# Caxson/mere-fusion

Hardware: AMD Instinct MI355X
Metric: lip-sync frames/sec @256x256 (higher is better)
Workload: dtype bf16x3+f16q; 1 GPU; MuseTalk step 256x256: pe(audio) + UNet(t=0) + VAE decode to uint8 frames, batch=8 latents + Whisper chunks per GPU, inputs resident in HBM (BASELINE.json configs[2]); assumed MuseTalk-v1 / sd-vae-ft-mse architecture, seeded random-init weights; batch_per_gpu=8, parallelism=1 independent replicas, sessions sharded by GPU, no collective

## Files before the change

include/merefusion.h:

```cpp
#ifndef MEREFUSION_H
#define MEREFUSION_H

#include <stddef.h>
#include <stdint.h>

#ifdef __cplusplus
extern "C" {
#endif

typedef enum mf_status {
    MF_OK = 0,
    MF_ERR_INVALID = -1,
    MF_ERR_HIP = -2,
    MF_ERR_NODEVICE = -3,
    MF_ERR_NOMEM = -4
} mf_status;

typedef enum mf_precision { MF_PREC_BF16 = 0, MF_PREC_BF16X3 = 1, MF_PREC_F16Q = 2 } mf_precision;

typedef struct mf_tensor {
    const char* name;
    const float* data;
    int ndim;
    int64_t shape[4];
// ... 35 lines not shown
    int transposed;
    int output_padding;
    int residual;
    int act;
    int in_h, in_w;
    int upsample;
    int pad_hi;
} mf_conv2d_desc;

int mf_conv2d_create(const mf_conv2d_desc* desc, const float* weight, const float* bias,
                     const float* bn_gamma, const float* bn_beta, const float* bn_mean,
                     const float* bn_var, int precision, mf_conv2d** out);
int mf_conv2d_forward(mf_conv2d* h, const float* x, float* y, int batch, void* stream);
int mf_conv2d_out_shape(const mf_conv2d* h, int* out_h, int* out_w);
int mf_conv2d_forward_stats(mf_conv2d* h, const float* x, float* y, int groups, double* stats, int batch, void* stream);
int mf_conv2d_time(mf_conv2d* h, int batch, int iters, float* ms, void* stream);
void mf_conv2d_destroy(mf_conv2d* h);
#define MF_CONV_FAMILY_IGEMM 0
#define MF_CONV_FAMILY_HALO 1
#define MF_CONV_FAMILY_HALO_W 2
#define MF_CONV_FAMILY_HALO_W_SPLIT 3
#define MF_CONV_FAMILY_TWIN 4
#define MF_CONV_FAMILY_THIN 5
#define MF_CONV_FAMILY_F16Q 6
#define MF_CONV_STATS_NONE 0
#define MF_CONV_STATS_EPILOGUE 1
#define MF_CONV_STATS_COMBINE 2
#define MF_CONV_STATS_PASS 3
int mf_conv2d_launch_config(const mf_conv2d* h, int batch, int stats_groups, int* info, int n);
int mf_conv2d_pin_config(mf_conv2d* h, int batch, int bm, int bn, int wgm, int wgn, int nsplit, int ld);
// ... 251 lines not shown
```

mere-fusion_amd/_lib.py:

```python
import ctypes as C
import os

HERE = os.path.dirname(os.path.abspath(__file__))
LIB_PATH = os.path.join(HERE, "libmerefusion_hip.so")

MF_PREC_BF16 = 0
MF_PREC_BF16X3 = 1
MF_PREC_F16Q = 2
PRECISIONS = {"bf16": MF_PREC_BF16, "bf16x3": MF_PREC_BF16X3, "f16q": MF_PREC_F16Q}


class MfTensor(C.Structure):
    _fields_ = [("name", C.c_char_p), ("data", C.c_void_p), ("ndim", C.c_int), ("shape", C.c_int64 * 4)]


class MfConv2dDesc(C.Structure):
    _fields_ = [(n, C.c_int) for n in (
        "cin", "cout", "kh", "kw", "stride_h", "stride_w", "pad_h", "pad_w", "transposed",
        "output_padding", "residual", "act", "in_h", "in_w", "upsample", "pad_hi")]


class MfUnetConfig(C.Structure):
    _fields_ = [("in_channels", C.c_int), ("out_channels", C.c_int), ("n_blocks", C.c_int),
                ("block_out_channels", C.c_int * 4), ("layers_per_block", C.c_int), ("cross_attention_dim", C.c_int),
# ... 51 lines not shown
    "mf_abi_version": (C.c_int, []),
    "mf_wav2lip_create": (C.c_int, [C.POINTER(MfTensor), C.c_int, C.c_int, C.POINTER(C.c_void_p)]),
    "mf_wav2lip_forward": (C.c_int, [C.c_void_p, C.c_void_p, C.c_void_p, C.c_void_p, C.c_int, C.c_void_p]),
    "mf_wav2lip_forward_u8": (C.c_int, [C.c_void_p, C.c_void_p, C.c_void_p, C.c_void_p, C.c_int, C.c_void_p]),
    "mf_wav2lip_read_tap": (C.c_int, [C.c_void_p, C.c_char_p, C.c_void_p, C.c_int, C.c_void_p]),
    "mf_wav2lip_num_launches": (C.c_int, [C.c_void_p, C.c_int]),
    "mf_wav2lip_launch_info": (C.c_int, [C.c_void_p, C.c_int, C.c_int, C.c_char_p, C.c_int, C.c_char_p, C.c_int,
                                        C.POINTER(C.c_double)]),
    "mf_wav2lip_profile": (C.c_int, [C.c_void_p, C.c_void_p, C.c_void_p, C.c_void_p, C.c_int, C.c_int,
                                     C.POINTER(C.c_float), C.c_void_p]),
    "mf_wav2lip_tune": (C.c_int, [C.c_void_p, C.c_int, C.c_void_p]),
    "mf_wav2lip_destroy": (None, [C.c_void_p]),
    "mf_conv2d_create": (C.c_int, [C.POINTER(MfConv2dDesc)] + [C.c_void_p] * 6 + [C.c_int, C.POINTER(C.c_void_p)]),
    "mf_conv2d_forward": (C.c_int, [C.c_void_p, C.c_void_p, C.c_void_p, C.c_int, C.c_void_p]),
    "mf_conv2d_forward_stats": (C.c_int, [C.c_void_p, C.c_void_p, C.c_void_p, C.c_int, C.c_void_p, C.c_int, C.c_void_p]),
    "mf_conv2d_out_shape": (C.c_int, [C.c_void_p, C.POINTER(C.c_int), C.POINTER(C.c_int)]),
    "mf_conv2d_time": (C.c_int, [C.c_void_p, C.c_int, C.c_int, C.POINTER(C.c_float), C.c_void_p]),
    "mf_conv2d_destroy": (None, [C.c_void_p]),
    "mf_conv2d_launch_config": (C.c_int, [C.c_void_p, C.c_int, C.c_int, C.POINTER(C.c_int), C.c_int]),
    "mf_conv2d_pin_config": (C.c_int, [C.c_void_p] + [C.c_int] * 7),
    "mf_whisper_create": (C.c_int, [C.POINTER(MfTensor), C.c_int, C.c_int, C.c_int, C.POINTER(C.c_void_p)]),
    "mf_whisper_dims": (C.c_int, [C.c_void_p, C.POINTER(C.c_int), C.POINTER(C.c_int), C.POINTER(C.c_int)]),
    "mf_whisper_log_mel": (C.c_int, [C.c_void_p, C.c_void_p, C.c_int, C.c_void_p, C.c_void_p]),
    "mf_whisper_encode_audio": (C.c_int, [C.c_void_p, C.c_void_p, C.c_int, C.c_void_p, C.c_void_p]),
    "mf_whisper_set_batch": (C.c_int, [C.c_void_p, C.c_int]),
    "mf_whisper_encode_windows": (C.c_int, [C.c_void_p, C.c_void_p, C.c_int, C.c_int, C.c_int, C.c_void_p, C.c_void_p]),
    "mf_whisper_destroy": (None, [C.c_void_p]),
    "mf_wav2vec2_create": (C.c_int, [C.POINTER(MfWav2Vec2Config), C.POINTER(MfTensor), C.c_int, C.c_int, C.c_int, C.c_int, C.POINTER(C.c_void_p)]),
    "mf_wav2vec2_frames": (C.c_int, [C.c_void_p, C.POINTER(C.c_int), C.POINTER(C.c_int)]),
    "mf_wav2vec2_forward": (C.c_int, [C.c_void_p, C.c_void_p, C.c_int, C.c_int, C.c_void_p, C.c_void_p]),
# ... 137 lines not shown
```

mere-fusion_amd/csrc/mf_conv.h:

```cpp
#pragma once
#include "mf_common.h"
#include <map>
#include <vector>
#include <utility>

struct ActBuf {
    int C = 0, H = 0, W = 0, halo = 0;
    bf16_t* hi = nullptr;
    bf16_t* lo = nullptr;
    int Hp() const { return H + 2 * halo; }
    int Wp() const { return W + 2 * halo; }
    int64_t per_batch() const { return (int64_t)Hp() * Wp() * C; }
};

struct ActView {
    const ActBuf* buf = nullptr;
    int coff = 0;
    int C = 0;
};

#define MF_MAX_PHASE 9

struct ConvPhase {
    int goff_begin;
// ... 13 lines not shown
    const int* goff;
    int M, N, Npad;
    int HqWq, Wq;
    uint32_t dv_hw_mul, dv_hw_shr, dv_w_mul, dv_w_shr;
    uint32_t dv_t_mul, dv_t_shr, dv_s_mul, dv_s_shr;
    int64_t xb; int xi, xj;
    int64_t yb; int yi, yj;
    int64_t rb; int ri, rj;
    int act;
    int res_after_act;
    int tiles_m, tiles_n;
    unsigned long long* dbg;
    int m_fastest;
    int ld;
    int wide_store;
    int goff_total;
    int zgroups, zheads;
    int64_t zx_b, zx_h, zw, zy_b, zy_h;
    float* ws;
    int64_t ws_split, wsb; int wsi, wsj;
    double* gn_out; int gn_out_cpg, gn_out_groups;
    double* ln_out; const double* ln_in; const float* ln_cs; float ln_inv_c, ln_eps;
    ConvPhase ph[MF_MAX_PHASE];
};

struct HaloArgs {
    const bf16_t* x_hi; const bf16_t* x_lo;
    const bf16_t* w_hi; const bf16_t* w_lo;
    const float* bias;
    const bf16_t* r_hi; const bf16_t* r_lo;
// ... 23 lines not shown
    int pad, in_halo, in_hp, in_wp, x_ld;
    int64_t xb, yb; int yi, yj;
    int act;
};
bool mf_thin_supported(int k, int stride, int cin, int cout);
int mf_thin_nks(int k, int cin);
void mf_thin_pack(const float* w, const float* scale, int cout, int cin, int k, bool x3, std::vector<bf16_t>& dst);
int mf_thin_launch(const ThinArgs& a, int k, int stride, int cin, int cout, bool x3, hipStream_t s);
HaloTile mf_halo_pick_tile(int H, int W, int N, int batch, int cin = 0);
int mf_halo_launch(const HaloArgs& a, const HaloTile& t, bool x3, hipStream_t s);
HaloTile mf_halo_w_pick_tile(int H, int W, int N, int batch, int cin = 0);
int mf_halo_w_launch(const HaloArgs& a, const HaloTile& t, bool x3, hipStream_t s, int phase = -1);
struct ConvTile { int bm, bn, wgm, wgn, nsplit; };
struct ConvTuned { ConvTile tile; int ld; };

struct ConvPlan {
    mf_conv2d_desc d{};
    int precision = 0;
    int cin_pad = 0;
    int out_h = 0, out_w = 0;
    int Hq = 0, Wq = 0;
    int nphase = 1;
    int Npad = 0;
    int BK = 64;
    bf16_t* w_hi = nullptr;
    bf16_t* w_lo = nullptr;
    float* bias = nullptr;
    int* goff = nullptr;
    double* out_stats = nullptr; int out_stats_groups = 0;
    const float* ln_gamma = nullptr; const float* ln_beta = nullptr;
    float* ln_cs = nullptr; const double* ln_in = nullptr; float ln_eps = 1e-5f;
    double* ln_out = nullptr;
// ... 22 lines not shown
    ConvPhase ph[MF_MAX_PHASE]{};
    int goff_total = 0;
    int bound_in_ld = -1, bound_in_wp = -1;
    std::map<int, ConvTuned> tuned;
};

int mf_conv_plan_create(ConvPlan* p, const mf_conv2d_desc& d, const float* weight, const float* bias,
                        const float* bn_gamma, const float* bn_beta, const float* bn_mean,
                        const float* bn_var, int precision);
void mf_conv_plan_destroy(ConvPlan* p);

int mf_conv_bind(ConvPlan* p, const ActBuf& in);

struct ConvLaunchCfg { int family; ConvTile tile; int ld, bk, nphase, stats; bool pinned; };
int mf_conv_resolve(const ConvPlan* p, int batch, int tokens, int stats_groups, ConvLaunchCfg* c);
bool mf_conv_tuned_valid(const ConvTuned& c, int precision, int act);
int mf_conv_pin(ConvPlan* p, int batch, const ConvTuned& c);
void mf_conv_kernel_name(const ConvPlan* p, int batch, char* buf, int cap);
ConvTile mf_conv_pick_tile(const ConvPlan* p, int batch);
int mf_conv_tune(ConvPlan* p, const ActView& in, const ActView& out, const ActView& res, int batch, hipStream_t stream);
int mf_conv_tune_lookup(ConvPlan* p, const ActView& in, int batch);
bool mf_autotune_enabled();
double mf_conv_flops(const ConvPlan* p, int batch);

struct GroupedGemm {
    const bf16_t* x_hi; const bf16_t* x_lo; int64_t zx_b, zx_h; int x_row;
    bf16_t* y_hi; bf16_t* y_lo; int64_t zy_b, zy_h; int y_row;
    int M, groups, heads;
};
int mf_gemm_grouped_launch(ConvPlan* p, const GroupedGemm& g, hipStream_t stream);
// ... 8 lines not shown
```

mere-fusion_amd/csrc/mf_conv.hip:

```cpp
#include "mf_conv.h"
#include <dlfcn.h>
#include <cmath>
#include <cstdlib>
#include <cstring>
#include <algorithm>
#include <map>
#include <set>
#include <string>
#include <type_traits>

typedef __attribute__((ext_vector_type(8))) __bf16 bf16x8;
typedef __attribute__((ext_vector_type(4))) float f32x4;
typedef __attribute__((ext_vector_type(4))) unsigned int u32x4;
typedef __attribute__((ext_vector_type(8))) _Float16 f16x8;
typedef __attribute__((ext_vector_type(8))) int i32x8;
typedef __attribute__((ext_vector_type(4))) int i32x4;

template <int BK>
__device__ __forceinline__ int swz(int row) {
    return BK == 32 ? (((row >> 2) & 1) << 1) : (((row >> 1) & 3) << 1);
}
template <int BK>
__device__ __forceinline__ int tile_off(int row, int kg) {
    return row * (BK * 2) + ((kg ^ swz<BK>(row)) << 4);
// ... 86 lines not shown
template <int BM, int BN, int BK, bool X3>
constexpr int igemm_ring() {
    constexpr int stage = (BM + BN) * BK * 2 * (X3 ? 2 : 1);
    constexpr int by_lds = (144 * 1024) / stage;
    return by_lds < 8 ? by_lds : 8;
}

#ifndef MF_PW_NPW
#define MF_PW_NPW 4
#endif
template <int BM, int BN, int BK>
constexpr int igemm_producers() {
    constexpr int rpc = 1024 / (BK * 2), pch = (BM + rpc - 1) / rpc, wch = (BN + rpc - 1) / rpc;
    return (pch % MF_PW_NPW == 0 && wch % MF_PW_NPW == 0) ? MF_PW_NPW : 4;
}
template <int BM, int BN, int WGM, int WGN, bool X3, int BK, int NST, int LD = 0, bool Q = false>
__global__ __launch_bounds__((WGM * WGN + (LD == 3 ? igemm_producers<BM, BN, BK>() : 0)) * 64) void k_conv_igemm(const ConvArgs a) {
    static_assert(!Q || X3, "the f16 + FP6 format has two planes");
    constexpr int NW = WGM * WGN;
    constexpr int NS = LD == 3 ? igemm_producers<BM, BN, BK>() : NW;
    constexpr int NT = (NW + (LD == 3 ? NS : 0)) * 64;
    static_assert(NW == 4 || NW == 8, "4 or 8 waves per workgroup");
    static_assert(BK == 32 || BK == 64, "LDS tile depth");
    static_assert(NST == 2, "two LDS stages (deeper rings halved the workgroups per CU and measured slower)");
    constexpr int KG = BK / 8;
    constexpr int ROWB = BK * 2;
    constexpr int RPC = 1024 / ROWB;
    constexpr int NP = X3 ? 2 : 1;
    constexpr int WTM = BM / WGM, WTN = BN / WGN;
    constexpr int FM = WTM / 16, FN = WTN / 16;
    static_assert(FM >= 1 && FN >= 1, "wave tile must hold a 16x16 fragment");
    constexpr int P_BYTES = BM * ROWB, W_BYTES = BN * ROWB;
    constexpr int PLANE = P_BYTES + W_BYTES;
// ... 150 lines not shown
#pragma unroll
                for (int j = 0; j < FM; ++j) {
                    if (X3) {
                        acc[i][j] = __builtin_amdgcn_mfma_f32_16x16x32_bf16(wf[NP - 1][i], pf[0][j], acc[i][j], 0, 0, 0);
                        acc[i][j] = __builtin_amdgcn_mfma_f32_16x16x32_bf16(wf[0][i], pf[NP - 1][j], acc[i][j], 0, 0, 0);
                    }
                    acc[i][j] = __builtin_amdgcn_mfma_f32_16x16x32_bf16(wf[0][i], pf[0][j], acc[i][j], 0, 0, 0);
                }
        }
    };
    auto compute = [&](int s) __attribute__((always_inline)) {
        const char* base = smem + s * STAGE;
        compute_at(base, PLANE, base + P_BYTES, PLANE);
    };

    __syncthreads();
    if (dbg && threadIdx.x == 0) dbg[1] = __builtin_amdgcn_s_memtime();
    const int nk = kt_end - kt_begin;
    if constexpr (LD == 3) {
        constexpr int NPI = (NPC + NWC) * NP;
        static_assert(PCH % NS == 0 && WCH >= NS, "producer-wave path: every producer issues the same number of pieces per stage (weight pieces: duplicates fill up)");
#ifndef MF_PW_LEAD
        constexpr int LEAD = DR >= 5 ? 2 : 1;
#else
        constexpr int LEAD = MF_PW_LEAD;
#endif
        static_assert((DR - 1 - LEAD) * NPI <= 63 && DR - 1 - LEAD >= 0, "vmcnt immediate");
        if (wave >= NW) {
            if (nk > 0) {
                const int pre = nk < DR - 1 ? nk : DR - 1;
                for (int d = 0; d < pre; ++d) stage(kt_begin + d, d);
                if (pre == DR - 1) wait_vm<(DR - 1 - LEAD) * NPI>(); else wait_vm<0>();
                __builtin_amdgcn_s_barrier();
// ... 27 lines not shown
        auto mma = [&](auto bufc) __attribute__((always_inline)) {
            constexpr int b = decltype(bufc)::value;
#pragma unroll
            for (int i = 0; i < FN; ++i)
#pragma unroll
                for (int j = 0; j < FM; ++j) {
                    if (X3) {
                        acc[i][j] = __builtin_amdgcn_mfma_f32_16x16x32_bf16(wfr[b][NP - 1][i], pfr[b][0][j], acc[i][j], 0, 0, 0);
                        acc[i][j] = __builtin_amdgcn_mfma_f32_16x16x32_bf16(wfr[b][0][i], pfr[b][NP - 1][j], acc[i][j], 0, 0, 0);
                    }
                    acc[i][j] = __builtin_amdgcn_mfma_f32_16x16x32_bf16(wfr[b][0][i], pfr[b][0][j], acc[i][j], 0, 0, 0);
                }
        };
        using B0 = std::integral_constant<int, 0>;
        using B1 = std::integral_constant<int, 1>;
        if (nk > 0 && LEAD == 1) {
            __syncthreads();
            int slot = 0;
            for (int i = 0; i < nk; ++i) {
                ldf(B0{}, slot, 0);
                if constexpr (KK == 2) ldf(B1{}, slot, 1);
                mma(B0{});
                if constexpr (KK == 2) mma(B1{});
                slot = slot + 1 == DR ? 0 : slot + 1;
                __syncthreads();
            }
        } else if (nk > 0) {
            __syncthreads();
            ldf(B0{}, 0, 0);
            int slot = 0;
// ... 14 lines not shown
                    mma(B0{});
                    slot = nslot;
                    __syncthreads();
                    if (i + 1 < nk) {
                        nslot = slot + 1 == DR ? 0 : slot + 1;
                        if (i + 2 < nk) ldf(B0{}, nslot, 0);
                        mma(B1{});
                        slot = nslot;
                        __syncthreads();
                    }
                }
            }
        }
    } else if constexpr (LD != 0) {
        static_assert(LD == 2, "register-staged tiles: one LDS stage");
        u32x4 rp[NP][NPC], rw[NP][NWC];
        auto gload = [&](int kt) __attribute__((always_inline)) {
#pragma unroll
            for (int i = 0; i < NPC; ++i) {
                const int c = wave + NW * i;
                if (PCH % NW == 0 || c < PCH) {
                    const bf16_t* src = xp[i] + s_goff[kt * KG + p_kg[i]];
                    rp[0][i] = *reinterpret_cast<const u32x4*>(src);
                    if (X3) rp[NP - 1][i] = *reinterpret_cast<const u32x4*>(src + x_delta);
                }
            }
#pragma unroll
            for (int i = 0; i < NWC; ++i) {
                const int c = wave + NW * i;
                if (WCH % NW == 0 || c < WCH) {
                    const bf16_t* src = BK == 64 ? wp[i] + kt * w_kstep : wp[i] + (kt >> 1) * w_kstep + (kt & 1) * 32;
                    rw[0][i] = *reinterpret_cast<const u32x4*>(src);
                    if (X3) rw[NP - 1][i] = *reinterpret_cast<const u32x4*>(src + w_delta);
                }
            }
        };
        auto lstore = [&](int s) __attribute__((always_inline)) {
            char* base = smem + s * STAGE + lane * 16;
#pragma unroll
            for (int i = 0; i < NPC; ++i) {
                const int c = wave + NW * i;
                if (PCH % NW == 0 || c < PCH) {
                    *reinterpret_cast<u32x4*>(base + c * 1024) = rp[0][i];
                    if (X3) *reinterpret_cast<u32x4*>(base + PLANE + c * 1024) = rp[NP - 1][i];
                }
            }
#pragma unroll
            for (int i = 0; i < NWC; ++i) {
                const int c = wave + NW * i;
                if (WCH % NW == 0 || c < WCH) {
                    *reinterpret_cast<u32x4*>(base + P_BYTES + c * 1024) = rw[0][i];
                    if (X3) *reinterpret_cast<u32x4*>(base + PLANE + P_BYTES + c * 1024) = rw[NP - 1][i];
                }
            }
        };
        {
            if (nk > 0) gload(kt_begin);
            for (int kt = kt_begin; kt < kt_end; ++kt) {
                if (kt > kt_begin) __syncthreads();
                lstore(0);
                if (kt + 1 < kt_end) gload(kt + 1);
                __syncthreads();
                compute(0);
            }
        }
    } else {
        if (nk > 0) {
            stage(kt_begin, 0);
            __syncthreads();
            for (int kt = kt_begin; kt < kt_end; ++kt) {
                const int s = (kt - kt_begin) & 1;
                if (kt + 1 < kt_end) stage(kt + 1, s ^ 1);
                compute(s);
                __syncthreads();
            }
        }
    }

    if (dbg && threadIdx.x == 0) dbg[2] = __builtin_amdgcn_s_memtime();
    if (a.ws) {
#pragma unroll
        for (int j = 0; j < FM; ++j) {
            const int m = m0 + pm0 + j * 16 + fr;
// ... 1 lines not shown
            const int b = mf_fdiv(m, a.dv_hw_mul, a.dv_hw_shr);
            const int rem = m - b * a.HqWq;
            const int qi = mf_fdiv(rem, a.dv_w_mul, a.dv_w_shr), qj = rem - qi * a.Wq;
            float* wo = a.ws + (int64_t)blockIdx.y * a.ws_split + (int64_t)b * a.wsb + (int64_t)qi * a.wsi +
                        (int64_t)qj * a.wsj + ph.ws_off;
#pragma unroll
            for (int i = 0; i < FN; ++i) {
                const int c = n0 + cn0 + i * 16 + fk * 4;
                if (c >= a.N) continue;
                *reinterpret_cast<float4*>(wo + c) = make_float4(acc[i][j][0], acc[i][j][1], acc[i][j][2], acc[i][j][3]);
            }
        }
        if (dbg && threadIdx.x == 0) dbg[3] = __builtin_amdgcn_s_memtime();
        return;
    }
    float4 bq[FN];
#pragma unroll
    for (int i = 0; i < FN; ++i) {
        int c = n0 + cn0 + i * 16 + fk * 4;
        c = c < a.Npad - 3 ? c : a.Npad - 4;
        bq[i] = *reinterpret_cast<const float4*>(a.bias + c);
    }
    const int ACT = a.act;
    if (a.ln_in) {
#pragma unroll
        for (int j = 0; j < FM; ++j) {
            const int m = m0 + pm0 + j * 16 + fr;
            const bool row_ok = m < a.M;
            const int mc = row_ok ? m : a.M - 1;
            const int b = mf_fdiv(mc, a.dv_hw_mul, a.dv_hw_shr);
            const int rem = mc - b * a.HqWq;
            const int qi = mf_fdiv(rem, a.dv_w_mul, a.dv_w_shr), qj = rem - qi * a.Wq;
            const int64_t yo = zy + (int64_t)b * a.yb + (int64_t)qi * a.yi + (int64_t)qj * a.yj + ph.y_off;
            const double2 sq = *reinterpret_cast<const double2*>(a.ln_in + 2 * (int64_t)mc);
            const double mean = sq.x * (double)a.ln_inv_c, var = sq.y * (double)a.ln_inv_c - mean * mean;
            const float mu = (float)mean, rs = (float)(1.0 / sqrt((var > 0.0 ? var : 0.0) + (double)a.ln_eps));
            auto quad = [&](int i, float (&v)[4]) __attribute__((always_inline)) {
                int c = n0 + cn0 + i * 16 + fk * 4;
                c = c < a.Npad - 3 ? c : a.Npad - 4;
                const float4 cs = *reinterpret_cast<const float4*>(a.ln_cs + c);
                float t0 = acc[i][j][0] - mu * cs.x, t1 = acc[i][j][1] - mu * cs.y, t2 = acc[i][j][2] - mu * cs.z, t3 = acc[i][j][3] - mu * cs.w;
                asm volatile("" : "+v"(t0), "+v"(t1), "+v"(t2), "+v"(t3));
                v[0] = rs * t0 + bq[i].x; v[1] = rs * t1 + bq[i].y; v[2] = rs * t2 + bq[i].z; v[3] = rs * t3 + bq[i].w;
                asm volatile("" : "+v"(v[0]), "+v"(v[1]), "+v"(v[2]), "+v"(v[3]));
            };
            auto pack = [&](const float (&v)[4], uint2& hi2, uint2& lo2) __attribute__((always_inline)) {
                uint32_t h[4];
#pragma unroll
                for (int e = 0; e < 4; ++e) h[e] = f2bf(v[e]);
                hi2 = make_uint2(h[0] | (h[1] << 16), h[2] | (h[3] << 16));
                if (X3) {
                    uint32_t l[4];
#pragma unroll
                    for (int e = 0; e < 4; ++e) l[e] = f2bf(v[e] - bf2f(h[e]));
                    lo2 = make_uint2(l[0] | (l[1] << 16), l[2] | (l[3] << 16));
// ... 101 lines not shown
        }
    } else {
        constexpr int RB = (FM * FN >= 32) ? 16 : 32;
        constexpr int JG = (FM * FN * NP <= RB) ? FM : (RB / (FN * NP) >= 1 ? RB / (FN * NP) : 1);
        const bool has_res = a.r_hi != nullptr;
        const bool after = a.res_after_act;
        constexpr bool ST = NW == 4 && FM * FN < 16;
        float gs[ST ? FN : 1][4], gq[ST ? FN : 1][4];
#pragma unroll
        for (int i = 0; i < (ST ? FN : 1); ++i)
#pragma unroll
            for (int e = 0; e < 4; ++e) { gs[i][e] = 0.f; gq[i][e] = 0.f; }
#pragma unroll
        for (int j0 = 0; j0 < FM; j0 += JG) {
            uint2 rh[JG][FN], rl[JG][FN];
            if (has_res) {
#pragma unroll
                for (int jj = 0; jj < JG; ++jj) {
                    if (j0 + jj >= FM) break;
                    int m = m0 + pm0 + (j0 + jj) * 16 + fr;
                    m = m < a.M ? m : a.M - 1;
                    const int b = mf_fdiv(m, a.dv_hw_mul, a.dv_hw_shr);
                    const int rem = m - b * a.HqWq;
                    const int qi = mf_fdiv(rem, a.dv_w_mul, a.dv_w_shr), qj = rem - qi * a.Wq;
                    const int64_t ro = (int64_t)b * a.rb + (int64_t)qi * a.ri + (int64_t)qj * a.rj;
#pragma unroll
                    for (int i = 0; i < FN; ++i) {
                        int c = n0 + cn0 + i * 16 + fk * 4;
                        c = c < a.N ? c : 0;
                        rh[jj][i] = *reinterpret_cast<const uint2*>(a.r_hi + ro + c);
                        if (X3) rl[jj][i] = *reinterpret_cast<const uint2*>(a.r_lo + ro + c);
// ... 330 lines not shown

static EpiDiv epi_div(const ConvArgs& e, int Ho, int Wo) {
    EpiDiv d{};
    const int nq = ((e.act == 5 ? e.N >> 1 : e.N) >> 2);
    const int nq_all = e.N >> 2, cols = nq_all < 256 ? nq_all : 256;
    mf_fastdiv((uint32_t)nq, &d.nq_mul, &d.nq_shr);
    mf_fastdiv((uint32_t)Wo, &d.w_mul, &d.w_shr);
    mf_fastdiv((uint32_t)Ho, &d.h_mul, &d.h_shr);
    mf_fastdiv((uint32_t)(e.gn_out_cpg > 0 ? e.gn_out_cpg : 1), &d.g_mul, &d.g_shr);
    mf_fastdiv((uint32_t)(cols > 0 ? cols : 1), &d.c_mul, &d.c_shr);
    return d;
}

namespace {

template <int BM, int BN, int WGM, int WGN, bool X3, int BK, int NST, int LD = 0, bool Q = false>
int launch_cfg_n(const ConvArgs& a, int nphase, int nsplit, int goff_max, hipStream_t s) {
    static bool attr_done = false;
    auto kern = k_conv_igemm<BM, BN, WGM, WGN, X3, BK, NST, LD, Q>;
    if (!attr_done) {
        MF_HIP(hipFuncSetAttribute(reinterpret_cast<const void*>(kern),
                                   hipFuncAttributeMaxDynamicSharedMemorySize, 160 * 1024));
        attr_done = true;
    }
    size_t lds = (size_t)(LD == 2 ? 1 : NST) * (BM + BN) * BK * 2 * (X3 ? 2 : 1) + (size_t)goff_max * 4;
    if constexpr (LD == 3) {
        lds = (size_t)igemm_ring<BM, BN, BK, X3>() * (BM + BN) * BK * 2 * (X3 ? 2 : 1) + (size_t)goff_max * 4;
        if (lds > 160 * 1024) { mf_set_error("conv: producer-wave tile %dx%d needs %zu bytes of LDS", BM, BN, lds); return MF_ERR_INVALID; }
    }
    dim3 grid(a.tiles_m * a.tiles_n, nsplit, a.zgroups ? a.zgroups : nphase);
    ConvArgs b = a;
    mf_fastdiv((uint32_t)(a.m_fastest ? a.tiles_m : a.tiles_n), &b.dv_t_mul, &b.dv_t_shr);
    mf_fastdiv((uint32_t)nsplit, &b.dv_s_mul, &b.dv_s_shr);
    hipLaunchKernelGGL(kern, grid, dim3((WGM * WGN + (LD == 3 ? igemm_producers<BM, BN, BK>() : 0)) * 64), lds, s, b);
// ... 890 lines not shown
    {
        const int n_out = p->d.act == 5 ? p->d.cout / 2 : p->d.cout;
        a.wide_store = out.coff % 8 == 0 && ob.C % 8 == 0 && n_out % 8 == 0 && p->d.cout % 16 == 0;
    }
    a.goff_total = p->goff_total;
    int goff_max = 0;
    for (int ph = 0; ph < p->nphase; ++ph) {
        a.ph[ph] = p->ph[ph];
        a.ph[ph].y_off = ((int64_t)p->phase_oy[ph] * ob.Wp() + p->phase_ox[ph]) * ob.C;
        a.ph[ph].ws_off = ((int64_t)p->phase_oy[ph] * p->out_w + p->phase_ox[ph]) * a.N;
        goff_max = std::max(goff_max, p->ph[ph].ngroups);
    }

    const ConvTile tc = cfg.tile;
    a.ld = cfg.ld;
    a.tiles_m = cdiv(a.M, tc.bm); a.tiles_n = cdiv(a.N, tc.bn);
    {
        const int64_t w_elems = (int64_t)a.Npad * p->ph[0].KT * 64 * p->nphase;
        const int64_t x_elems = (int64_t)batch * ib.H * ib.W * in.C;
        a.m_fastest = w_elems > x_elems;
        static const bool dbg_times = mf_debug_has("times");
        if (dbg_times) {
            static unsigned long long* dbg_buf = nullptr;
            if (!dbg_buf) MF_HIP(hipMalloc(&dbg_buf, (size_t)4 * 65536 * sizeof(unsigned long long)));
            a.dbg = (int64_t)a.tiles_m * a.tiles_n * tc.nsplit * p->nphase <= 65536 ? dbg_buf : nullptr;
        }
    }
    if (tc.nsplit > 1) {
        const int64_t per_split = (int64_t)batch * p->out_h * out_w_eff * a.N;
        const int64_t need = per_split * tc.nsplit;
// ... 50 lines not shown
    }
    if (tc.nsplit > 1 && p->prof_mid) MF_HIP(hipEventRecord(p->prof_mid, stream));
    if (tc.nsplit > 1) {
        ConvArgs e = a;
        e.yi = ob.Wp() * ob.C; e.yj = ob.C;
        const int64_t total = (int64_t)batch * p->out_h * out_w_eff * ((a.act == 5 ? a.N / 2 : a.N) / 4);
        MF_REQUIRE(total < 0x7fffffffll, "conv: split-K combine over %lld channel quads (32-bit thread index)", (long long)total);
        if (tokens == 0 && launch_combine_stats(p, e, tc.nsplit, p->out_h, out_w_eff, batch, stream)) *stats_done = true;
        else hipLaunchKernelGGL(k_splitk_epilogue, dim3((unsigned)((total + 255) / 256)), dim3(256), 0, stream, e,
                                tc.nsplit, p->out_h, out_w_eff, (int)total, epi_div(e, p->out_h, out_w_eff));
        MF_HIP(hipGetLastError());
    }
    return MF_OK;
}

int mf_gemm_grouped_launch(ConvPlan* p, const GroupedGemm& g, hipStream_t stream) {
    MF_REQUIRE(!p->halo && p->nphase == 1 && p->bound_in_ld > 0, "grouped gemm: plan must be a bound mf_gemm_plan_create shell");
    const bool x3 = p->precision == MF_PREC_BF16X3;
    ConvArgs a{};
    a.x_hi = g.x_hi; a.x_lo = x3 ? g.x_lo : nullptr;
    a.w_hi = p->w_hi; a.w_lo = p->w_lo; a.bias = p->bias; a.goff = p->goff;
    a.M = g.M; a.N = p->d.cout; a.Npad = p->Npad;
    a.HqWq = g.M; a.Wq = g.M;
    mf_fastdiv((uint32_t)a.HqWq, &a.dv_hw_mul, &a.dv_hw_shr); mf_fastdiv((uint32_t)a.Wq, &a.dv_w_mul, &a.dv_w_shr);
    a.xb = 0; a.xi = 0; a.xj = g.x_row;
    a.y_hi = g.y_hi; a.y_lo = x3 ? g.y_lo : nullptr;
    a.yb = 0; a.yi = 0; a.yj = g.y_row;
    a.act = 0;
    a.ld = -1;
    a.goff_total = p->goff_total;
    a.ph[0] = p->ph[0];
    a.zgroups = g.groups; a.zheads = g.heads;
    a.zx_b = g.zx_b; a.zx_h = g.zx_h; a.zy_b = g.zy_b; a.zy_h = g.zy_h;
    a.zw = (int64_t)p->ph[0].KT * p->Npad * 64;
    const int M = g.M, N = a.N;
    int rc = MF_ERR_INVALID;
#define MF_GCASE(BM, BN, WGM, WGN)                                                         \
    { a.tiles_m = cdiv(M, BM); a.tiles_n = cdiv(N, BN);                                    \
      rc = launch_prec<BM, BN, WGM, WGN>(a, 1, 1, p->ph[0].ngroups, x3, false, stream); }
    if (N <= 16) MF_GCASE(128, 16, 4, 1)
    else if (N <= 32) MF_GCASE(128, 32, 4, 1)
    else if (M <= 16) MF_GCASE(16, 64, 1, 4)
    else if (cdiv(M, 128) * cdiv(N, 128) * g.groups >= 512 && N % 128 == 0) MF_GCASE(128, 128, 2, 2)
    else if (cdiv(M, 128) * cdiv(N, 64) * g.groups >= 512) MF_GCASE(128, 64, 2, 2)
// ... 302 lines not shown
```

mere-fusion_amd/csrc/mf_conv_api.hip:

```cpp
#include "mf_conv.h"
#include "mf_aux.h"
#include <memory>
#include <algorithm>

static int out_channels(const mf_conv2d_desc& d) { return d.act == 5 ? d.cout / 2 : d.cout; }

struct mf_conv2d {
    ConvPlan plan;
    ActBuf in, out;
    int cap = 0;
    ~mf_conv2d() {
        mf_conv_plan_destroy(&plan);
        for (ActBuf* b : {&in, &out}) {
            if (b->hi) (void)hipFree(b->hi);
            if (b->lo) (void)hipFree(b->lo);
        }
    }
};

extern "C" int mf_conv2d_create(const mf_conv2d_desc* desc, const float* weight, const float* bias,
                                const float* bn_gamma, const float* bn_beta, const float* bn_mean,
                                const float* bn_var, int precision, mf_conv2d** out) {
    MF_REQUIRE(desc && weight && out, "conv2d_create: null argument");
    MF_REQUIRE((bn_gamma != nullptr) == (bn_beta != nullptr) && (bn_gamma != nullptr) == (bn_mean != nullptr) &&
// ... 42 lines not shown
    ActView res = h->plan.d.residual ? ActView{&h->in, 0, h->plan.d.cout} : ActView{};
    if ((rc = mf_conv_launch(&h->plan, in, out, res, batch, s))) return rc;
    return mf_act_to_nchw(out, y, batch, s);
}

extern "C" int mf_conv2d_forward_stats(mf_conv2d* h, const float* x, float* y, int groups, double* stats, int batch, void* stream) {
    MF_REQUIRE(h && stats && groups > 0 && groups <= 64 && h->plan.d.act != 5 && h->plan.d.cout % groups == 0 && h->plan.d.cout % 8 == 0,
               "conv2d_forward_stats: needs cout %% groups == 0, cout %% 8 == 0, groups <= 64, no GEGLU");
    MF_HIP(hipMemsetAsync(stats, 0, (size_t)batch * groups * 2 * sizeof(double), (hipStream_t)stream));
    h->plan.out_stats = stats; h->plan.out_stats_groups = groups;
    const int rc = mf_conv2d_forward(h, x, y, batch, stream);
    h->plan.out_stats = nullptr; h->plan.out_stats_groups = 0;
    return rc;
}

extern "C" int mf_conv2d_time(mf_conv2d* h, int batch, int iters, float* ms, void* stream) {
    MF_REQUIRE(h && ms, "conv2d_time: null argument");
    MF_REQUIRE(batch > 0 && batch <= h->cap && iters > 0, "conv2d_time: run mf_conv2d_forward at this batch first");
    hipStream_t s = (hipStream_t)stream;
    ActView in{&h->in, 0, h->in.C}, out{&h->out, 0, out_channels(h->plan.d)};
    ActView res = h->plan.d.residual ? ActView{&h->in, 0, h->plan.d.cout} : ActView{};
    hipEvent_t e0, e1;
    MF_HIP(hipEventCreate(&e0)); MF_HIP(hipEventCreate(&e1));
    MF_HIP(hipEventRecord(e0, s));
    for (int i = 0; i < iters; ++i) {
        int rc = mf_conv_launch(&h->plan, in, out, res, batch, s);
        if (rc) return rc;
    }
    MF_HIP(hipEventRecord(e1, s));
    MF_HIP(hipEventSynchronize(e1));
// ... 6 lines not shown

extern "C" int mf_conv2d_out_shape(const mf_conv2d* h, int* out_h, int* out_w) {
    MF_REQUIRE(h && out_h && out_w, "conv2d_out_shape: null argument");
    *out_h = h->plan.out_h; *out_w = h->plan.out_w;
    return MF_OK;
}

extern "C" void mf_conv2d_destroy(mf_conv2d* h) { delete h; }

extern "C" int mf_conv2d_launch_config(const mf_conv2d* h, int batch, int stats_groups, int* info, int n) {
    MF_REQUIRE(h && info && n >= 11 && batch > 0 && stats_groups >= 0, "conv2d_launch_config: needs a handle, batch > 0, stats_groups >= 0 and room for 11 ints");
    ConvLaunchCfg c;
    if (const int rc = mf_conv_resolve(&h->plan, batch, 0, stats_groups, &c)) return rc;
    const int v[11] = {c.family, c.tile.bm, c.tile.bn, c.tile.wgm, c.tile.wgn, c.tile.nsplit, c.ld, c.bk, c.nphase, c.stats, c.pinned ? 1 : 0};
    std::copy(v, v + 11, info);
    return MF_OK;
}

extern "C" int mf_conv2d_pin_config(mf_conv2d* h, int batch, int bm, int bn, int wgm, int wgn, int nsplit, int ld) {
    MF_REQUIRE(h && batch > 0, "conv2d_pin_config: null handle or batch <= 0");
    return mf_conv_pin(&h->plan, batch, ConvTuned{ConvTile{bm, bn, wgm, wgn, nsplit}, ld});
}
```

Baseline: 452.4 frames/s.

## Prefetch epilogue operands during the igemm mainloop and split register-staged loads

Adds an EPF variant of the implicit-GEMM conv kernel that loads bias, layernorm statistics and residual tiles into registers during the last mainloop stage, so the epilogue no longer waits on those global loads. For register-staged (LD==2) forms it also issues the first weight load before the initial barrier and splits activation and weight loads. The variant is enabled by default through an env switch and is limited to 4-wave forms with small fragment counts. It raises register pressure, which may cut occupancy. New LN-conv API entry points are added for testing.

```diff
diff --git a/include/merefusion.h b/include/merefusion.h
--- a/include/merefusion.h
+++ b/include/merefusion.h
@@ -73,6 +73,9 @@
 int mf_conv2d_forward(mf_conv2d* h, const float* x, float* y, int batch, void* stream);
 int mf_conv2d_out_shape(const mf_conv2d* h, int* out_h, int* out_w);
 int mf_conv2d_forward_stats(mf_conv2d* h, const float* x, float* y, int groups, double* stats, int batch, void* stream);
+int mf_conv2d_create_ln(const mf_conv2d_desc* desc, const float* weight, const float* bias, const float* ln_gamma, const float* ln_beta, float eps,
+                        int precision, mf_conv2d** out);
+int mf_conv2d_forward_ln(mf_conv2d* h, const float* x, const double* stats, float* y, int batch, void* stream);
 int mf_conv2d_time(mf_conv2d* h, int batch, int iters, float* ms, void* stream);
 void mf_conv2d_destroy(mf_conv2d* h);
 #define MF_CONV_FAMILY_IGEMM 0
diff --git a/mere-fusion_amd/_lib.py b/mere-fusion_amd/_lib.py
--- a/mere-fusion_amd/_lib.py
+++ b/mere-fusion_amd/_lib.py
@@ -89,6 +89,8 @@
     "mf_conv2d_create": (C.c_int, [C.POINTER(MfConv2dDesc)] + [C.c_void_p] * 6 + [C.c_int, C.POINTER(C.c_void_p)]),
     "mf_conv2d_forward": (C.c_int, [C.c_void_p, C.c_void_p, C.c_void_p, C.c_int, C.c_void_p]),
     "mf_conv2d_forward_stats": (C.c_int, [C.c_void_p, C.c_void_p, C.c_void_p, C.c_int, C.c_void_p, C.c_int, C.c_void_p]),
+    "mf_conv2d_create_ln": (C.c_int, [C.POINTER(MfConv2dDesc)] + [C.c_void_p] * 4 + [C.c_float, C.c_int, C.POINTER(C.c_void_p)]),
+    "mf_conv2d_forward_ln": (C.c_int, [C.c_void_p, C.c_void_p, C.c_void_p, C.c_void_p, C.c_int, C.c_void_p]),
     "mf_conv2d_out_shape": (C.c_int, [C.c_void_p, C.POINTER(C.c_int), C.POINTER(C.c_int)]),
     "mf_conv2d_time": (C.c_int, [C.c_void_p, C.c_int, C.c_int, C.POINTER(C.c_float), C.c_void_p]),
     "mf_conv2d_destroy": (None, [C.c_void_p]),
diff --git a/mere-fusion_amd/csrc/mf_conv.h b/mere-fusion_amd/csrc/mf_conv.h
--- a/mere-fusion_amd/csrc/mf_conv.h
+++ b/mere-fusion_amd/csrc/mf_conv.h
@@ -1,5 +1,6 @@
 #pragma once
 #include "mf_common.h"
+#include <cstdlib>
 #include <map>
 #include <vector>
 #include <utility>
@@ -51,6 +52,7 @@
     int m_fastest;
     int ld;
     int wide_store;
+    int epi_pf;
     int goff_total;
     int zgroups, zheads;
     int64_t zx_b, zx_h, zw, zy_b, zy_h;
@@ -104,8 +106,11 @@
 struct ConvTile { int bm, bn, wgm, wgn, nsplit; };
 struct ConvTuned { ConvTile tile; int ld; };
 
+inline bool mf_epi_prefetch_env() { const char* e = getenv("MF_EPI_PREFETCH"); return !(e && *e && atoi(e) == 0); }
+
 struct ConvPlan {
     mf_conv2d_desc d{};
+    bool epi_prefetch = mf_epi_prefetch_env();
     int precision = 0;
     int cin_pad = 0;
     int out_h = 0, out_w = 0;
@@ -158,6 +163,7 @@
 
 struct ConvLaunchCfg { int family; ConvTile tile; int ld, bk, nphase, stats; bool pinned; };
 int mf_conv_resolve(const ConvPlan* p, int batch, int tokens, int stats_groups, ConvLaunchCfg* c);
+bool mf_conv_epf_runs(const ConvPlan* p, const ConvLaunchCfg& c);
 bool mf_conv_tuned_valid(const ConvTuned& c, int precision, int act);
 int mf_conv_pin(ConvPlan* p, int batch, const ConvTuned& c);
 void mf_conv_kernel_name(const ConvPlan* p, int batch, char* buf, int cap);
diff --git a/mere-fusion_amd/csrc/mf_conv.hip b/mere-fusion_amd/csrc/mf_conv.hip
--- a/mere-fusion_amd/csrc/mf_conv.hip
+++ b/mere-fusion_amd/csrc/mf_conv.hip
@@ -124,9 +124,16 @@
     constexpr int rpc = 1024 / (BK * 2), pch = (BM + rpc - 1) / rpc, wch = (BN + rpc - 1) / rpc;
     return (pch % MF_PW_NPW == 0 && wch % MF_PW_NPW == 0) ? MF_PW_NPW : 4;
 }
-template <int BM, int BN, int WGM, int WGN, bool X3, int BK, int NST, int LD = 0, bool Q = false>
+constexpr bool igemm_epf_form(int bm, int bn, int wgm, int wgn, bool x3, int bk, int ld, bool q) {
+    return wgm * wgn == 4 && !q && (bm / wgm / 16) * (bn / wgn / 16) <= 8 && !(ld == 2 && !x3 && bm == 128 && bn == 64) && !(ld != 3 && x3 && bk == 32);
+}
+template <int BM, int BN, int WGM, int WGN, bool X3, int BK, int LD, bool Q>
+constexpr bool igemm_epf() { return igemm_epf_form(BM, BN, WGM, WGN, X3, BK, LD, Q); }
+
+template <int BM, int BN, int WGM, int WGN, bool X3, int BK, int NST, int LD = 0, bool Q = false, bool EPF = false>
 __global__ __launch_bounds__((WGM * WGN + (LD == 3 ? igemm_producers<BM, BN, BK>() : 0)) * 64) void k_conv_igemm(const ConvArgs a) {
     static_assert(!Q || X3, "the f16 + FP6 format has two planes");
+    static_assert(!EPF || igemm_epf<BM, BN, WGM, WGN, X3, BK, LD, Q>(), "epilogue operand prefetch: forms that keep their workgroups per CU only");
     constexpr int NW = WGM * WGN;
     constexpr int NS = LD == 3 ? igemm_producers<BM, BN, BK>() : NW;
     constexpr int NT = (NW + (LD == 3 ? NS : 0)) * 64;
@@ -307,9 +314,83 @@
         compute_at(base, PLANE, base + P_BYTES, PLANE);
     };
 
+    float4 bq[FN];
+    constexpr int PF_LN = 4 * FM + 4 * FN, PF_RES = 2 * FM * FN * NP;
+    uint32_t pf[EPF ? (PF_LN > PF_RES ? PF_LN : PF_RES) : 1];
+    static_assert(!EPF || FM * FN * NP <= 16, "the prefetched residual is one row group of the general epilogue");
+    auto epi_prefetch = [&]() __attribute__((always_inline)) {
+        if constexpr (EPF) {
+            if (a.ws) return;
+#pragma unroll
+            for (int i = 0; i < FN; ++i) {
+                int c = n0 + cn0 + i * 16 + fk * 4;
+                c = c < a.Npad - 3 ? c : a.Npad - 4;
+                bq[i] = *reinterpret_cast<const float4*>(a.bias + c);
+                if (a.ln_in) {
+                    const uint4 cs = *reinterpret_cast<const uint4*>(a.ln_cs + c);
+                    pf[4 * FM + 4 * i] = cs.x; pf[4 * FM + 4 * i + 1] = cs.y; pf[4 * FM + 4 * i + 2] = cs.z; pf[4 * FM + 4 * i + 3] = cs.w;
+                }
+            }
+            if (a.ln_in) {
+#pragma unroll
+                for (int j = 0; j < FM; ++j) {
+                    const int m = m0 + pm0 + j * 16 + fr;
+                    const int mc = m < a.M ? m : a.M - 1;
+                    const uint4 sq = *reinterpret_cast<const uint4*>(a.ln_in + 2 * (int64_t)mc);
+                    pf[4 * j] = sq.x; pf[4 * j + 1] = sq.y; pf[4 * j + 2] = sq.z; pf[4 * j + 3] = sq.w;
+                }
+            } else if (a.r_hi && !(FN % 2 == 0 && a.act == 5)) {
+#pragma unroll
+                for (int j = 0; j < FM; ++j) {
+                    int m = m0 + pm0 + j * 16 + fr;
+                    m = m < a.M ? m : a.M - 1;
+                    const int b = mf_fdiv(m, a.dv_hw_mul, a.dv_hw_shr);
+                    const int rem = m - b * a.HqWq;
+                    const int qi = mf_fdiv(rem, a.dv_w_mul, a.dv_w_shr), qj = rem - qi * a.Wq;
+                    const int64_t ro = (int64_t)b * a.rb + (int64_t)qi * a.ri + (int64_t)qj * a.rj;
+#pragma unroll
+                    for (int i = 0; i < FN; ++i) {
+                        int c = n0 + cn0 + i * 16 + fk * 4;
+                        c = c < a.N ? c : 0;
+                        const uint2 h = *reinterpret_cast<const uint2*>(a.r_hi + ro + c);
+                        pf[2 * (j * FN + i)] = h.x; pf[2 * (j * FN + i) + 1] = h.y;
+                        if (X3) {
+                            const uint2 l = *reinterpret_cast<const uint2*>(a.r_lo + ro + c);
+                            pf[2 * (FM * FN + j * FN + i)] = l.x; pf[2 * (FM * FN + j * FN + i) + 1] = l.y;
+                        }
+                    }
+                }
+            }
+        }
+    };
+    u32x4 rp[NP][LD == 2 ? NPC : 1], rw[NP][LD == 2 ? NWC : 1];
+    auto gload_p = [&](int kt) __attribute__((always_inline)) {
+#pragma unroll
+        for (int i = 0; i < NPC; ++i) {
+            const int c = wave + NW * i;
+            if (PCH % NW == 0 || c < PCH) {
+                const bf16_t* src = xp[i] + s_goff[kt * KG + p_kg[i]];
+                rp[0][i] = *reinterpret_cast<const u32x4*>(src);
+                if (X3) rp[NP - 1][i] = *reinterpret_cast<const u32x4*>(src + x_delta);
+            }
+        }
+    };
+    auto gload_w = [&](int kt) __attribute__((always_inline)) {
+#pragma unroll
+        for (int i = 0; i < NWC; ++i) {
+            const int c = wave + NW * i;
+            if (WCH % NW == 0 || c < WCH) {
+                const bf16_t* src = BK == 64 ? wp[i] + kt * w_kstep : wp[i] + (kt >> 1) * w_kstep + (kt & 1) * 32;
+                rw[0][i] = *reinterpret_cast<const u32x4*>(src);
+                if (X3) rw[NP - 1][i] = *reinterpret_cast<const u32x4*>(src + w_delta);
+            }
+        }
+    };
+    const int nk = kt_end - kt_begin;
+    if constexpr (EPF && LD == 2) { if (nk > 0) gload_w(kt_begin); }
+
     __syncthreads();
     if (dbg && threadIdx.x == 0) dbg[1] = __builtin_amdgcn_s_memtime();
-    const int nk = kt_end - kt_begin;
     if constexpr (LD == 3) {
         constexpr int NPI = (NPC + NWC) * NP;
         static_assert(PCH % NS == 0 && WCH >= NS, "producer-wave path: every producer issues the same number of pieces per stage (weight pieces: duplicates fill up)");
@@ -367,6 +448,7 @@
         };
         using B0 = std::integral_constant<int, 0>;
         using B1 = std::integral_constant<int, 1>;
+        epi_prefetch();
         if (nk > 0 && LEAD == 1) {
             __syncthreads();
             int slot = 0;
@@ -411,27 +493,6 @@
         }
     } else if constexpr (LD != 0) {
         static_assert(LD == 2, "register-staged tiles: one LDS stage");
-        u32x4 rp[NP][NPC], rw[NP][NWC];
-        auto gload = [&](int kt) __attribute__((always_inline)) {
-#pragma unroll
-            for (int i = 0; i < NPC; ++i) {
-                const int c = wave + NW * i;
-                if (PCH % NW == 0 || c < PCH) {
-                    const bf16_t* src = xp[i] + s_goff[kt * KG + p_kg[i]];
-                    rp[0][i] = *reinterpret_cast<const u32x4*>(src);
-                    if (X3) rp[NP - 1][i] = *reinterpret_cast<const u32x4*>(src + x_delta);
-                }
-            }
-#pragma unroll
-            for (int i = 0; i < NWC; ++i) {
-                const int c = wave + NW * i;
-                if (WCH % NW == 0 || c < WCH) {
-                    const bf16_t* src = BK == 64 ? wp[i] + kt * w_kstep : wp[i] + (kt >> 1) * w_kstep + (kt & 1) * 32;
-                    rw[0][i] = *reinterpret_cast<const u32x4*>(src);
-                    if (X3) rw[NP - 1][i] = *reinterpret_cast<const u32x4*>(src + w_delta);
-                }
-            }
-        };
         auto lstore = [&](int s) __attribute__((always_inline)) {
             char* base = smem + s * STAGE + lane * 16;
 #pragma unroll
@@ -451,19 +512,38 @@
                 }
             }
         };
-        {
-            if (nk > 0) gload(kt_begin);
+        if constexpr (EPF) {
+            if (nk > 0) gload_p(kt_begin);
+            for (int kt = kt_begin; kt + 1 < kt_end; ++kt) {
+                if (kt > kt_begin) __syncthreads();
+                lstore(0);
+                gload_p(kt + 1); gload_w(kt + 1);
+                __syncthreads();
+                compute(0);
+            }
+            if (nk > 0) {
+                if (nk > 1) __syncthreads();
+                lstore(0);
+                epi_prefetch();
+                __syncthreads();
+                compute(0);
+            } else {
+                epi_prefetch();
+            }
+        } else {
+            if (nk > 0) { gload_p(kt_begin); gload_w(kt_begin); }
             for (int kt = kt_begin; kt < kt_end; ++kt) {
                 if (kt > kt_begin) __syncthreads();
                 lstore(0);
-                if (kt + 1 < kt_end) gload(kt + 1);
+                if (kt + 1 < kt_end) { gload_p(kt + 1); gload_w(kt + 1); }
                 __syncthreads();
                 compute(0);
             }
         }
     } else {
+        if (nk > 0) stage(kt_begin, 0);
+        epi_prefetch();
         if (nk > 0) {
-            stage(kt_begin, 0);
             __syncthreads();
             for (int kt = kt_begin; kt < kt_end; ++kt) {
                 const int s = (kt - kt_begin) & 1;
@@ -495,12 +575,13 @@
         if (dbg && threadIdx.x == 0) dbg[3] = __builtin_amdgcn_s_memtime();
         return;
     }
-    float4 bq[FN];
-#pragma unroll
-    for (int i = 0; i < FN; ++i) {
-        int c = n0 + cn0 + i * 16 + fk * 4;
-        c = c < a.Npad - 3 ? c : a.Npad - 4;
-        bq[i] = *reinterpret_cast<const float4*>(a.bias + c);
+    if constexpr (!EPF) {
+#pragma unroll
+        for (int i = 0; i < FN; ++i) {
+            int c = n0 + cn0 + i * 16 + fk * 4;
+            c = c < a.Npad - 3 ? c : a.Npad - 4;
+            bq[i] = *reinterpret_cast<const float4*>(a.bias + c);
+        }
     }
     const int ACT = a.act;
     if (a.ln_in) {
@@ -513,13 +594,17 @@
             const int rem = mc - b * a.HqWq;
             const int qi = mf_fdiv(rem, a.dv_w_mul, a.dv_w_shr), qj = rem - qi * a.Wq;
             const int64_t yo = zy + (int64_t)b * a.yb + (int64_t)qi * a.yi + (int64_t)qj * a.yj + ph.y_off;
-            const double2 sq = *reinterpret_cast<const double2*>(a.ln_in + 2 * (int64_t)mc);
+            double2 sq;
+            if constexpr (EPF) { sq.x = __hiloint2double((int)pf[4 * j + 1], (int)pf[4 * j]); sq.y = __hiloint2double((int)pf[4 * j + 3], (int)pf[4 * j + 2]); }
+            else sq = *reinterpret_cast<const double2*>(a.ln_in + 2 * (int64_t)mc);
             const double mean = sq.x * (double)a.ln_inv_c, var = sq.y * (double)a.ln_inv_c - mean * mean;
             const float mu = (float)mean, rs = (float)(1.0 / sqrt((var > 0.0 ? var : 0.0) + (double)a.ln_eps));
             auto quad = [&](int i, float (&v)[4]) __attribute__((always_inline)) {
                 int c = n0 + cn0 + i * 16 + fk * 4;
                 c = c < a.Npad - 3 ? c : a.Npad - 4;
-                const float4 cs = *reinterpret_cast<const float4*>(a.ln_cs + c);
+                float4 cs;
+                if constexpr (EPF) cs = make_float4(__uint_as_float(pf[4 * FM + 4 * i]), __uint_as_float(pf[4 * FM + 4 * i + 1]), __uint_as_float(pf[4 * FM + 4 * i + 2]), __uint_as_float(pf[4 * FM + 4 * i + 3]));
+                else cs = *reinterpret_cast<const float4*>(a.ln_cs + c);
                 float t0 = acc[i][j][0] - mu * cs.x, t1 = acc[i][j][1] - mu * cs.y, t2 = acc[i][j][2] - mu * cs.z, t3 = acc[i][j][3] - mu * cs.w;
                 asm volatile("" : "+v"(t0), "+v"(t1), "+v"(t2), "+v"(t3));
                 v[0] = rs * t0 + bq[i].x; v[1] = rs * t1 + bq[i].y; v[2] = rs * t2 + bq[i].z; v[3] = rs * t3 + bq[i].w;
@@ -651,7 +736,18 @@
 #pragma unroll
         for (int j0 = 0; j0 < FM; j0 += JG) {
             uint2 rh[JG][FN], rl[JG][FN];
-            if (has_res) {
+            if constexpr (EPF) {
+                static_assert(JG == FM, "one row group");
+                if (has_res) {
+#pragma unroll
+                    for (int jj = 0; jj < FM; ++jj)
+#pragma unroll
+                        for (int i = 0; i < FN; ++i) {
+                            rh[jj][i] = make_uint2(pf[2 * (jj * FN + i)], pf[2 * (jj * FN + i) + 1]);
+                            if (X3) rl[jj][i] = make_uint2(pf[2 * (FM * FN + jj * FN + i)], pf[2 * (FM * FN + jj * FN + i) + 1]);
+                        }
+                }
+            } else if (has_res) {
 #pragma unroll
                 for (int jj = 0; jj < JG; ++jj) {
                     if (j0 + jj >= FM) break;
@@ -1012,10 +1108,13 @@
 
 namespace {
 
-template <int BM, int BN, int WGM, int WGN, bool X3, int BK, int NST, int LD = 0, bool Q = false>
+template <int BM, int BN, int WGM, int WGN, bool X3, int BK, int NST, int LD = 0, bool Q = false, bool EPF = false>
 int launch_cfg_n(const ConvArgs& a, int nphase, int nsplit, int goff_max, hipStream_t s) {
+    if constexpr (!EPF && igemm_epf<BM, BN, WGM, WGN, X3, BK, LD, Q>()) {
+        if (a.epi_pf && !a.ws) return launch_cfg_n<BM, BN, WGM, WGN, X3, BK, NST, LD, Q, true>(a, nphase, nsplit, goff_max, s);
+    }
     static bool attr_done = false;
-    auto kern = k_conv_igemm<BM, BN, WGM, WGN, X3, BK, NST, LD, Q>;
+    auto kern = k_conv_igemm<BM, BN, WGM, WGN, X3, BK, NST, LD, Q, EPF>;
     if (!attr_done) {
         MF_HIP(hipFuncSetAttribute(reinterpret_cast<const void*>(kern),
                                    hipFuncAttributeMaxDynamicSharedMemorySize, 160 * 1024));
@@ -1936,6 +2035,7 @@
 
     const ConvTile tc = cfg.tile;
     a.ld = cfg.ld;
+    a.epi_pf = p->epi_prefetch;
     a.tiles_m = cdiv(a.M, tc.bm); a.tiles_n = cdiv(a.N, tc.bn);
     {
         const int64_t w_elems = (int64_t)a.Npad * p->ph[0].KT * 64 * p->nphase;
@@ -2016,6 +2116,11 @@
     return MF_OK;
 }
 
+bool mf_conv_epf_runs(const ConvPlan* p, const ConvLaunchCfg& c) {
+    if ((c.family != MF_CONV_FAMILY_IGEMM && c.family != MF_CONV_FAMILY_TWIN) || !p->epi_prefetch || c.tile.nsplit > 1) return false;
+    return igemm_epf_form(c.tile.bm, c.tile.bn, c.tile.wgm, c.tile.wgn, p->precision != MF_PREC_BF16, c.bk, c.ld >= 3 ? 3 : c.ld, p->q);
+}
+
 int mf_gemm_grouped_launch(ConvPlan* p, const GroupedGemm& g, hipStream_t stream) {
     MF_REQUIRE(!p->halo && p->nphase == 1 && p->bound_in_ld > 0, "grouped gemm: plan must be a bound mf_gemm_plan_create shell");
     const bool x3 = p->precision == MF_PREC_BF16X3;
@@ -2030,6 +2135,7 @@
     a.yb = 0; a.yi = 0; a.yj = g.y_row;
     a.act = 0;
     a.ld = -1;
+    a.epi_pf = p->epi_prefetch;
     a.goff_total = p->goff_total;
     a.ph[0] = p->ph[0];
     a.zgroups = g.groups; a.zheads = g.heads;
diff --git a/mere-fusion_amd/csrc/mf_conv_api.hip b/mere-fusion_amd/csrc/mf_conv_api.hip
--- a/mere-fusion_amd/csrc/mf_conv_api.hip
+++ b/mere-fusion_amd/csrc/mf_conv_api.hip
@@ -80,6 +80,29 @@
     return rc;
 }
 
+extern "C" int mf_conv2d_create_ln(const mf_conv2d_desc* desc, const float* weight, const float* bias, const float* ln_gamma, const float* ln_beta, float eps,
+                                   int precision, mf_conv2d** out) {
+    MF_REQUIRE(desc && weight && ln_gamma && ln_beta && out, "conv2d_create_ln: null argument");
+    *out = nullptr;
+    std::unique_ptr<mf_conv2d> h(new mf_conv2d());
+    h->plan.ln_gamma = ln_gamma; h->plan.ln_beta = ln_beta; h->plan.ln_eps = eps;
+    int rc = mf_conv_plan_create(&h->plan, *desc, weight, bias, nullptr, nullptr, nullptr, nullptr, precision);
+    if (rc) return rc;
+    h->in.C = h->plan.cin_pad; h->in.H = desc->in_h; h->in.W = desc->in_w; h->in.halo = std::max(1, h->plan.in_halo_need);
+    h->out.C = (out_channels(*desc) + 7) / 8 * 8; h->out.H = h->plan.out_h; h->out.W = h->plan.out_w; h->out.halo = 1;
+    if ((rc = mf_conv_bind(&h->plan, h->in))) return rc;
+    *out = h.release();
+    return MF_OK;
+}
+
+extern "C" int mf_conv2d_forward_ln(mf_conv2d* h, const float* x, const double* stats, float* y, int batch, void* stream) {
+    MF_REQUIRE(h && stats && h->plan.ln_cs, "conv2d_forward_ln: needs a layer of mf_conv2d_create_ln and its statistics");
+    h->plan.ln_in = stats;
+    const int rc = mf_conv2d_forward(h, x, y, batch, stream);
+    h->plan.ln_in = nullptr;
+    return rc;
+}
+
 extern "C" int mf_conv2d_time(mf_conv2d* h, int batch, int iters, float* ms, void* stream) {
     MF_REQUIRE(h && ms, "conv2d_time: null argument");
     MF_REQUIRE(batch > 0 && batch <= h->cap && iters > 0, "conv2d_time: run mf_conv2d_forward at this batch first");
@@ -116,6 +139,7 @@
     if (const int rc = mf_conv_resolve(&h->plan, batch, 0, stats_groups, &c)) return rc;
     const int v[11] = {c.family, c.tile.bm, c.tile.bn, c.tile.wgm, c.tile.wgn, c.tile.nsplit, c.ld, c.bk, c.nphase, c.stats, c.pinned ? 1 : 0};
     std::copy(v, v + 11, info);
+    if (n >= 12) info[11] = mf_conv_epf_runs(&h->plan, c) ? 1 : 0;
     return MF_OK;
 }
 
```

Result: no change. 453.4 frames/s (median of 2 runs) (+0.2%).
